# chanzuckerberg/saber

Hardware: AMD Instinct MI355X
Metric: EM slices/sec (1024^2, Hiera-L) (higher is better)
Workload: dtype bf16; 1 GPU; 1024x1024 uint16 EM slice -> prep.prepare -> SAM2 AMG (Hiera-L, cfgAMG defaults: npoints=32, crop_n_layers=2 -> 21 crops, 3072 grid prompts + 9216 m2m refinements, multimask) -> dedup/sort -> uint16 label plane; BASELINE configs[1]; weights=seeded synthetic Hiera-L (no checkpoint offline), slices_per_rank=22, engine_handles_per_gpu=2, parallelism=single GPU

## Files before the change

include/saber_amd_kernels.h:

```cpp
#ifndef SABER_AMD_KERNELS_H
#define SABER_AMD_KERNELS_H
#include <stddef.h>
#include <stdint.h>
#ifdef __cplusplus
extern "C" {
#endif

const char* saber_k_last_error(void);
int saber_k_init(int device_id);

int saber_k_gemm(const uint16_t* A, const uint16_t* W, const float* bias, const float* res, float* out_f32, uint16_t* out_bf16,
                 int M, int N, int K, int act, int act_last, int pool4, int res_shift, int res_mod, void* stream);

int saber_k_gemm_ld(const uint16_t* A, int lda, const uint16_t* W, int ldw, int w_kpad, const float* bias, const float* res, float* out_f32,
                    uint16_t* out_bf16, int M, int N, int K, int act, void* stream);

int saber_k_gemm_rowln(const uint16_t* A, int lda, const uint16_t* W, int ldw, const float* bias, const float* res, float* out_f32,
                       uint16_t* out_bf16, const float* ln_gamma, const float* ln_beta, float ln_eps, uint16_t* ln_out, int M, int N, int K,
                       void* stream);

int saber_k_mlp_rowln(const uint16_t* A, int lda, const uint16_t* W1, int ldw1, const float* b1, const uint16_t* W2, int ldw2, const float* b2,
                      const float* res, float* out_f32, uint16_t* out_bf16, const float* ln_gamma, const float* ln_beta, float ln_eps,
                      uint16_t* ln_out, int M, int C, void* stream);

// ... 1 lines not shown
                      int rows, int C, int act, void* stream);

int saber_k_hiera_attention(const uint16_t* qkv, uint16_t* out, int n_windows, int nk, int heads, int q_pool, void* stream);
int saber_k_hiera_attention_ex(const uint16_t* qkv, uint16_t* out, int n_windows, int nk, int heads, int head_dim, int q_pool,
                               const uint8_t* key_mask, void* stream);

int saber_k_dec_attention(const float* q, const float* k, const float* v, uint16_t* out, int B, int nq, int nk, int heads, int hd,
                          int k_shared, void* stream);

int saber_k_prepare(const void* img, int dtype, int H, int W, float* out, float* ws_dev, uint32_t* minmax_dev, void* stream);

int saber_k_mask_post(const float* lowres, int n, int crop_x0, int crop_y0, int crop_w, int crop_h, int H, int W, float thr,
                      float offset, uint32_t* bits, int32_t* stats, void* stream);
int saber_k_mask_post_ex(const float* lowres, const int* idx, const uint8_t* pass, int n, int crop_x0, int crop_y0, int crop_w, int crop_h,
                         int H, int W, float thr, float offset, uint32_t* bits, int32_t* stats, void* stream);

int saber_k_resize_normalize(const float* img, int H, int W, int channels, const int* crops_dev, int n, float* out, int res, void* stream);
int saber_k_patch_embed(const float* pix, const float* wt, const float* bias, const float* pos, float* out, int n_images, int C, void* stream);

int saber_k_rope(const float* x, int64_t rows, int n_rot, int C, int side, float theta, float* out_f32, uint16_t* out_bf16, void* stream);
int saber_k_softmax_rows(const float* S, int64_t ld_s, int64_t rows, int n, float scale, uint16_t* P, int64_t ld_p, void* stream);
int saber_k_conv3x3s2(const float* in, int H, int W, int Cin, const float* w, const float* b, int Cout, float* out, void* stream);
int saber_k_conv3x3s2_t(const float* in, int H, int W, int Cin, const float* wt, const float* b, int Cout, float* out, void* stream);
int saber_k_paint_nearest(const float* logits, int Hv, int Wv, float thr, int label, uint16_t* plane, int H, int W, int* any_flag, void* stream);
int saber_k_paint_nearest_stack(const float* logits, int n, int Hv, int Wv, const int* labels_host, float thr, uint16_t* plane, int H, int W,
                                int* any_flag, void* stream);
int saber_k_relabel_frames(uint16_t* vol, int Z, int64_t HW, const uint16_t* lut, int L, void* stream);
int saber_k_merge_max_u16(uint16_t* acc, const uint16_t* src, int64_t n, int binarize, void* stream);
int saber_k_merge_class_conf(uint16_t* final_labels, float* best, const uint16_t* src, const uint16_t* cls, const float* conf, int L, int64_t n,
                             void* stream);
// ... 105 lines not shown
```

saber_amd/_lib.py:

```python
import ctypes as C
import os
import subprocess

_HERE = os.path.dirname(os.path.abspath(__file__))
LIB_PATH = os.path.join(_HERE, "libsaber_amd.so")
CSRC = os.path.join(_HERE, "csrc")


class SaberAmdError(RuntimeError):
    pass


class SaberRangeError(SaberAmdError):
    """SABER_ERR_RANGE: the engine's overflow sentinel found NaN / inf in the 16-bit arithmetic (include/saber_amd.h:
    saber_engine_check_finite) - with fp16 operands, an activation beyond 65 504.  The call's results are invalid."""


SABER_OK, SABER_ERR_INVALID, SABER_ERR_STATE, SABER_ERR_HIP, SABER_ERR_CAPACITY, SABER_ERR_RANGE = 0, -1, -2, -3, -4, -5


def build(verbose: bool = False) -> str:
    r = subprocess.run(["make", "-C", CSRC, "-j8"], capture_output=True, text=True)
    if r.returncode != 0:
        raise SaberAmdError("building libsaber_amd.so failed:\n" + r.stdout[-4000:] + r.stderr[-4000:])
# ... 105 lines not shown
    "saber_encoder_flops": (C.c_double, [_vp]),
    "saber_decoder_flops_per_prompt": (C.c_double, []),
    "saber_k_last_error": (C.c_char_p, []),
    "saber_k_init": (_i, [_i]),
    "saber_k_gemm": (_i, [_vp, _vp, _vp, _vp, _vp, _vp, _i, _i, _i, _i, _i, _i, _i, _i, _vp]),
    "saber_k_gemm_ld": (_i, [_vp, _i, _vp, _i, _i, _vp, _vp, _vp, _vp, _i, _i, _i, _i, _vp]),
    "saber_k_gemm_rowln": (_i, [_vp, _i, _vp, _i, _vp, _vp, _vp, _vp, _vp, _vp, _f, _vp, _i, _i, _i, _vp]),
    "saber_k_mlp_rowln": (_i, [_vp, _i, _vp, _i, _vp, _vp, _i, _vp, _vp, _vp, _vp, _vp, _vp, _f, _vp, _i, _i, _vp]),
    "saber_k_layernorm": (_i, [_vp, _vp, _vp, _f, _vp, _vp, _i, _i, _i, _vp]),
    "saber_k_hiera_attention": (_i, [_vp, _vp, _i, _i, _i, _i, _vp]),
    "saber_k_hiera_attention_ex": (_i, [_vp, _vp, _i, _i, _i, _i, _i, _vp, _vp]),
    "saber_k_dec_attention": (_i, [_vp, _vp, _vp, _vp, _i, _i, _i, _i, _i, _i, _vp]),
    "saber_k_prepare": (_i, [_vp, _i, _i, _i, _vp, _vp, _vp, _vp]),
    "saber_k_mask_post": (_i, [_vp, _i, _i, _i, _i, _i, _i, _i, _f, _f, _vp, _vp, _vp]),
    "saber_k_mask_post_ex": (_i, [_vp, _vp, _vp, _i, _i, _i, _i, _i, _i, _i, _f, _f, _vp, _vp, _vp]),
    "saber_k_resize_normalize": (_i, [_vp, _i, _i, _i, _vp, _i, _vp, _i, _vp]),
    "saber_k_patch_embed": (_i, [_vp, _vp, _vp, _vp, _vp, _i, _i, _vp]),
    "saber_k_perm_index": (_i, [_i, _i, _i]),
    "saber_k_set_operand_type": (_i, [_i]),
    "saber_k_stream_create_cu_range": (_i, [_i, _i, C.POINTER(_vp)]),
    "saber_k_stream_destroy": (_i, [_vp]),
    "saber_k_host_f32_to_f16": (None, [_vp, _vp, C.c_int64]),
    "saber_k_dec_i2t": (_i, [_vp, C.c_int64, _vp, _vp, _vp, _f, _vp, _vp, _vp, _vp, _vp, _f, _vp, _i, _vp]),
    "saber_k_dec_i2t16": (_i, [_vp, C.c_int64, _vp, _vp, _vp, _f, _vp, _vp, _vp, _vp, _vp, _f, _vp, _i, _i, _vp]),
    "saber_k_dec_t2i": (_i, [_vp, C.c_int64, _vp, _vp, _vp, _f, _vp, _vp, _i, _i, _vp, _vp, _vp, _vp]),
    "saber_k_dec_upscale": (_i, [_vp, _vp, _vp, _vp, _vp, _vp, _vp, _vp, _vp, _i, _i, _vp, _vp, _i, _vp, _vp, _i, _vp, _vp]),
    "saber_k_hyper_pack": (_i, [_vp, _i, _vp, _vp, _vp]),
    "saber_k_mask_pick": (_i, [_vp, _vp, _i, _i, _vp, _vp, _vp, _vp]),
    "saber_k_mask_select": (_i, [_vp, _vp, _i, _i, _vp, _vp, _vp]),
    "saber_k_iou_live_flags": (_i, [_vp, _i, _f, _vp, _vp, _vp]),
# ... 79 lines not shown
```

saber_amd/csrc/amg.hip:

```cpp
#include <algorithm>
#include <array>
#include <cmath>
#include <numeric>

#include "common.h"
#include "engine.h"

#define TRY(x) do { int _r = (x); if (_r != SABER_OK) return _r; } while (0)

struct Cand {
    float box[4];
    float iou, stab;
    float pt[2];
    int crop[4];
    int area;
    size_t bits_slot;
};

static std::vector<int> nms_host(const std::vector<Cand>& c, const std::vector<float>& scores, float thr) {
    const int n = (int)c.size();
    std::vector<int> order(n);
    std::iota(order.begin(), order.end(), 0);
    std::stable_sort(order.begin(), order.end(), [&](int a, int b) { return scores[a] > scores[b]; });
    std::vector<char> sup(n, 0);
// ... 238 lines not shown
            if (prm->use_m2m) {
                float* pts2 = e->amg_pts2 + 2 * gr.k0;
                float* low2 = e->amg_low2 + gr.k0 * 4 * 65536;
                float* iou2 = e->amg_iou2 + gr.k0;
                int* sel2 = e->amg_sel + gr.k0;
                TRY(eng_graphed(e, "dec2," + key_of({ci, nm, (long long)(uintptr_t)pts2, G * nm, first_raw, (long long)(uintptr_t)low1, (long long)(uintptr_t)low2, (long long)(uintptr_t)iou2, (long long)(uintptr_t)sel2,
                                                     (long long)(e->iou_prune ? std::lround(prm->pred_iou_thresh * 1e6f) + 1 : 0)}), s,
                                [&]() { return eng_decode_ex(e, ci, nm, pts2, nullptr, G * nm, 0, low1, first_raw, 32.0f, low2, 1, iou2, nullptr, sel2, s, prm->pred_iou_thresh); }));
                for (int g = 0; g < G; ++g) e->slot_embb_valid[ci + g] = 1;
                gr.masks = low2; gr.ious = iou2; gr.plane_mode = 2;
            }
        }
        if (use_dev) {
            const float* iou_all = prm->use_m2m ? e->amg_iou2 : e->amg_iou1;
            std::vector<DevCrop> dcs;
            for (const Grp& gr : groups) {
                ENG_KP(e, PC_ELEMENTWISE, 0.0, 0.0, launch_amg_plane(iou_all + gr.k0, gr.plane_mode == 2 ? e->amg_sel + gr.k0 : nullptr, gr.G * gr.nm, gr.plane_mode, prm->pred_iou_thresh,
                                                                  e->amg_idx + gr.k0, e->amg_pass + gr.k0, s));
                if (lowres_clean)
                    ENG_KP(e, PC_MASK_POST, 0.0, 0.0, launch_clean_lowres(const_cast<float*>(gr.masks), e->amg_idx + gr.k0, e->amg_pass + gr.k0, gr.G * gr.nm, 256, 256, prm->mask_threshold,
                                                                         e->lowres_hole_area, e->lowres_sprinkle_area, s));
                for (int g = 0; g < gr.G; ++g) {
                    const auto& box = crops[c0 + gr.ci + g];
                    DevCrop dc{{box[0], box[1], box[2], box[3]}, (int)(gr.k0 + (size_t)g * gr.nm), gr.nm, (int)(gr.pt0 + (size_t)g * gr.np), M};
                    dcs.push_back(dc);
                    ENG_KP(e, PC_MASK_POST, 0.0, (double)gr.nm * (65536.0 * 4 + (double)mask_words * 4),
                           launch_mask_post(gr.masks, e->amg_idx + dc.kbase, gr.nm, box[0], box[1], box[2] - box[0], box[3] - box[1], H, W, prm->mask_threshold,
                                            prm->stability_score_offset, e->amg_crop_bits + (slot_base + dc.kbase) * mask_words, e->amg_stats + dc.kbase, s, e->amg_pass + dc.kbase));
                }
            }
            ENG_HIP(e, hipMemcpyAsync(e->amg_crops_dev, dcs.data(), sizeof(DevCrop) * dcs.size(), hipMemcpyHostToDevice, s));
            ENG_HIP(e, hipMemcpyAsync(e->amg_crop_pts, crop_pts_all.data(), sizeof(float) * 2 * n_pts, hipMemcpyHostToDevice, s));
            ENG_KP(e, PC_MASK_POST, 0.0, 0.0, launch_amg_crops(e->amg_crops_dev, (int)dcs.size(), max_nm, e->amg_stats, e->amg_pass, iou_all, e->amg_crop_pts, prm->stability_score_thresh,
                                                            prm->box_nms_thresh, H, W, (int)slot_base, e->amg_tmp, e->amg_keep, e->amg_counts, e->amg_surv, e->amg_nsurv, (int)total_cand, s));
            slot_base += n_cand;
            continue;
        }
        std::vector<float> h_iou_all(n_cand);
        std::vector<int> h_sel;
        ENG_HIP(e, hipMemcpyAsync(h_iou_all.data(), prm->use_m2m ? e->amg_iou2 : e->amg_iou1, sizeof(float) * n_cand, hipMemcpyDeviceToHost, s));
        if (prm->use_m2m) { h_sel.resize(n_cand); ENG_HIP(e, hipMemcpyAsync(h_sel.data(), e->amg_sel, sizeof(int) * n_cand, hipMemcpyDeviceToHost, s)); }
        { ENG_HIP(e, hipStreamSynchronize(s)); ++e->amg_last_syncs; }
        struct CropRange { int first, count; };
        std::vector<std::vector<CropRange>> ranges(groups.size());
        h_idx.clear();
        for (size_t gi = 0; gi < groups.size(); ++gi) {
// ... 165 lines not shown
```

saber_amd/csrc/capi_kernels.hip:

```cpp
#include <cmath>
#include <cstring>
#include <string>
#include <vector>

#include "../../include/saber_amd_kernels.h"
#include "common.h"
#include "kernels.h"
#include "engine.h"
#include "exact.h"

#include <atomic>

static thread_local std::string g_kerr;
static int kfail(const char* m) { g_kerr = m ? m : "unknown"; return -1; }
static int kcheck(const char* m) {
    if (m) return kfail(m);
    hipError_t st = hipGetLastError();
    if (st != hipSuccess) return kfail(hipGetErrorString(st));
    return 0;
}

extern "C" const char* saber_k_last_error(void) { return g_kerr.c_str(); }

extern "C" int saber_k_init(int device_id) {
// ... 104 lines not shown
    if (dtype == 0) return kcheck(launch_prepare_u16((const uint16_t*)img, H, W, out, ws_dev, minmax_dev, (hipStream_t)stream));
    if (dtype == 1) return kcheck(launch_prepare_f32((const float*)img, H, W, out, ws_dev, minmax_dev, (hipStream_t)stream));
    return kfail("prepare: dtype must be 0 (u16) or 1 (f32)");
}

extern "C" int saber_k_mask_post(const float* lowres, int n, int crop_x0, int crop_y0, int crop_w, int crop_h, int H, int W, float thr,
                                 float offset, uint32_t* bits, int32_t* stats, void* stream) {
    return kcheck(launch_mask_post(lowres, nullptr, n, crop_x0, crop_y0, crop_w, crop_h, H, W, thr, offset, bits,
                                   reinterpret_cast<MaskStats*>(stats), (hipStream_t)stream));
}

extern "C" int saber_k_mask_post_ex(const float* lowres, const int* idx, const uint8_t* pass, int n, int crop_x0, int crop_y0, int crop_w, int crop_h,
                                    int H, int W, float thr, float offset, uint32_t* bits, int32_t* stats, void* stream) {
    return kcheck(launch_mask_post(lowres, idx, n, crop_x0, crop_y0, crop_w, crop_h, H, W, thr, offset, bits,
                                   reinterpret_cast<MaskStats*>(stats), (hipStream_t)stream, pass));
}

extern "C" int saber_k_resize_normalize(const float* img, int H, int W, int channels, const int* crops_dev, int n, float* out, int res, void* stream) {
    if (res <= 0 || (res % 16) != 0) return kfail("resize_normalize: res must be a positive multiple of 16");
    if (n <= 0) return 0;
    return kcheck(launch_resize_normalize(img, H, W, channels, crops_dev, n, out, res, (hipStream_t)stream));
}

extern "C" int saber_k_patch_embed(const float* pix, const float* wt, const float* bias, const float* pos, float* out, int n_images, int C, void* stream) {
    if (n_images <= 0) return 0;
    return kcheck(launch_patch_embed(pix, wt, bias, pos, out, n_images, C, 1024, (hipStream_t)stream));
}

extern "C" int saber_k_perm_index(int y, int x, int stage) { return perm_index(y, x, stage); }

// ... 327 lines not shown
```

saber_amd/csrc/decoder_ops.hip:

```cpp
#include <algorithm>

#include "common.h"
#include "kernels.h"

#define DEC_C 256

__global__ __launch_bounds__(256) void prompt_tokens_kernel(const float* __restrict__ pts, const int* __restrict__ labels, int P,
                                                            PromptWeights w, float* __restrict__ tokens) {
    const int p = blockIdx.x, c = threadIdx.x;
    float* t = tokens + (int64_t)p * 8 * DEC_C;
#pragma unroll
    for (int k = 0; k < 6; ++k) t[k * DEC_C + c] = w.out_tokens[k * DEC_C + c];
    const int label = labels ? labels[p] : 1;
    float e = 0.f;
    if (label >= 0) {
        const float x = 2.0f * ((pts[2 * p] + 0.5f) / 1024.0f) - 1.0f;
        const float y = 2.0f * ((pts[2 * p + 1] + 0.5f) / 1024.0f) - 1.0f;
        const int f = c & 127;
        const float a = 6.283185307179586f * (x * w.gauss[f] + y * w.gauss[128 + f]);
        e = (c < 128 ? sinf(a) : cosf(a)) + w.point_embed[(label & 3) * DEC_C + c];
    } else {
        e = w.not_a_point[c];
    }
    t[6 * DEC_C + c] = e;
// ... 691 lines not shown
        for (int w = 0; w < 4; ++w) {
            a += red[w][0]; in_ += red[w][1]; u += red[w][2];
            x0 = min(x0, red[w][3]); x1 = max(x1, red[w][4]); y0 = min(y0, red[w][5]); y1 = max(y1, red[w][6]);
        }
        MaskStats* st = stats + mi;
        if (a) {
            atomicAdd(&st->area, a);
            atomicMin(&st->x0, x0); atomicMax(&st->x1, x1);
            atomicMin(&st->y0, y0); atomicMax(&st->y1, y1);
        }
        if (in_) atomicAdd(&st->inter, in_);
        if (u) atomicAdd(&st->uni, u);
    }
}

__global__ __launch_bounds__(256) void mask_post_w1k_kernel(const float* __restrict__ lowres, const int* __restrict__ idx, int crop_x0,
                                                            int crop_y0, int crop_w, int crop_h, int H, int W, float thr, float offset,
                                                            uint32_t* __restrict__ bits, MaskStats* __restrict__ stats, const uint8_t* __restrict__ pass) {
    if (pass && !pass[blockIdx.y]) return;
    __shared__ float vrow[4][260];
    __shared__ int red[4][8];
    const int mi = blockIdx.y;
    const float* src = lowres + (int64_t)(idx ? idx[mi] : mi) * 65536;
    const int lane = threadIdx.x & 63, wave = threadIdx.x >> 6;
    const int W32 = (W + 31) >> 5;
    const float sy_scale = 256.0f / (float)crop_h, sx_scale = 256.0f / (float)crop_w;
    const int c_lo = max(crop_x0, 0) >> 6, c_hi = min(crop_x0 + crop_w - 1, W - 1) >> 6;
    int x0a[16];
    float lxa[16];
#pragma unroll
    for (int c = 0; c < 16; ++c) {
        const int x = 64 * c + lane, cx = x - crop_x0;
        float sx = ((float)cx + 0.5f) * sx_scale - 0.5f;
        sx = fmaxf(sx, 0.f);
        const int x0i = min((int)sx, 255);
        const bool valid = x < W && cx >= 0 && cx < crop_w;
        x0a[c] = valid ? x0i : 257;
        lxa[c] = valid ? sx - (float)x0i : 0.0f;
    }
    if (lane < 2) vrow[wave][257 + lane] = -3.0e38f;
    auto fetch = [&](int y, float4* a, float4* b, float* ly) -> bool {
        const int cy = y - crop_y0;
        if (y >= H || cy < 0 || cy >= crop_h) return false;
        float sy = ((float)cy + 0.5f) * sy_scale - 0.5f;
        sy = fmaxf(sy, 0.f);
        const int y0i = min((int)sy, 255), y1i = min(y0i + 1, 255);
        *ly = sy - (float)y0i;
        *a = *reinterpret_cast<const float4*>(src + y0i * 256 + lane * 4);
        *b = *reinterpret_cast<const float4*>(src + y1i * 256 + lane * 4);
        return true;
    };
    int area = 0, inter = 0, uni = 0, xmin = 1 << 30, xmax = -1, ymin = 1 << 30, ymax = -1;
    const int ybase = blockIdx.x * MP_ROWS + wave * (MP_ROWS / 4);
    float4 na = make_float4(0.f, 0.f, 0.f, 0.f), nb = na;
    float nly = 0.f;
    bool nin = fetch(ybase, &na, &nb, &nly);
    for (int r = 0; r < MP_ROWS / 4; ++r) {
        const int y = ybase + r;
        if (y >= H) break;
        uint32_t* brow = bits + ((int64_t)mi * H + y) * W32;
        const float4 a = na, b = nb;
        const float ly = nly;
        const bool in_crop = nin;
        nin = (r + 1 < MP_ROWS / 4) ? fetch(y + 1, &na, &nb, &nly) : false;
        if (!in_crop) {
            for (int wd = lane; wd < W32; wd += 64) brow[wd] = 0u;
            continue;
        }
        __builtin_amdgcn_wave_barrier();
        {
            float* vw = vrow[wave] + lane * 4;
            vw[0] = (1.0f - ly) * a.x + ly * b.x; vw[1] = (1.0f - ly) * a.y + ly * b.y;
            vw[2] = (1.0f - ly) * a.z + ly * b.z; vw[3] = (1.0f - ly) * a.w + ly * b.w;
            if (lane == 63) vw[4] = vw[3];
        }
        __builtin_amdgcn_wave_barrier();
        const float* vr = vrow[wave];
        uint32_t blo = 0u, bhi = 0u;
        float ta[16], tb[16];
#pragma unroll
        for (int cc = 0; cc < 16; ++cc) { ta[cc] = vr[x0a[cc]]; tb[cc] = vr[x0a[cc] + 1]; }
#define MP_CHUNK(cc)                                                                                              \
        if ((cc) >= c_lo && (cc) <= c_hi) {                                                                       \
            const float lx = lxa[cc];                                                                             \
            const float v = (1.0f - lx) * ta[cc] + lx * tb[cc];                                                   \
            const unsigned long long bm = __ballot(v > thr);                                                      \
            asm("s_nop 1\n\tv_writelane_b32 %0, %1, " #cc : "+v"(blo) : "s"((uint32_t)bm));     \
            asm("v_writelane_b32 %0, %1, " #cc : "+v"(bhi) : "s"((uint32_t)(bm >> 32)));                          \
            inter += (v > thr + offset) ? 1 : 0;                                                                  \
            uni += (v > thr - offset) ? 1 : 0;                                                                    \
        }
        MP_CHUNK(0) MP_CHUNK(1) MP_CHUNK(2) MP_CHUNK(3) MP_CHUNK(4) MP_CHUNK(5) MP_CHUNK(6) MP_CHUNK(7)
        MP_CHUNK(8) MP_CHUNK(9) MP_CHUNK(10) MP_CHUNK(11) MP_CHUNK(12) MP_CHUNK(13) MP_CHUNK(14) MP_CHUNK(15)
#undef MP_CHUNK
        const int pc = __popc(blo) + __popc(bhi);
        area += pc;
        if (pc) {
            xmin = min(xmin, lane * 64 + (blo ? __ffs((int)blo) - 1 : 31 + __ffs((int)bhi)));
            xmax = max(xmax, lane * 64 + (bhi ? 63 - __clz((int)bhi) : 31 - __clz((int)blo)));
        }
        if (__ballot(pc != 0)) { ymin = min(ymin, y); ymax = max(ymax, y); }
        const int wd = lane * 2;
        if (wd < W32) brow[wd] = blo;
        if (wd + 1 < W32) brow[wd + 1] = bhi;
    }
#pragma unroll
    for (int o = 32; o > 0; o >>= 1) {
        area += __shfl_xor(area, o, 64); inter += __shfl_xor(inter, o, 64); uni += __shfl_xor(uni, o, 64);
        xmin = min(xmin, __shfl_xor(xmin, o, 64)); xmax = max(xmax, __shfl_xor(xmax, o, 64));
    }
    if (lane == 0) {
        red[wave][0] = area; red[wave][1] = inter; red[wave][2] = uni; red[wave][3] = xmin;
        red[wave][4] = xmax; red[wave][5] = ymin; red[wave][6] = ymax;
    }
    __syncthreads();
    if (threadIdx.x == 0) {
        int a = 0, in_ = 0, u = 0, x0 = 1 << 30, x1 = -1, y0 = 1 << 30, y1 = -1;
        for (int w = 0; w < 4; ++w) {
            a += red[w][0]; in_ += red[w][1]; u += red[w][2];
            x0 = min(x0, red[w][3]); x1 = max(x1, red[w][4]); y0 = min(y0, red[w][5]); y1 = max(y1, red[w][6]);
        }
        MaskStats* st = stats + mi;
        if (a) {
            atomicAdd(&st->area, a);
            atomicMin(&st->x0, x0); atomicMax(&st->x1, x1);
            atomicMin(&st->y0, y0); atomicMax(&st->y1, y1);
        }
        if (in_) atomicAdd(&st->inter, in_);
        if (u) atomicAdd(&st->uni, u);
    }
}

__global__ void mask_stats_init_kernel(MaskStats* stats, int n) {
    const int i = blockIdx.x * 256 + threadIdx.x;
    if (i < n) { MaskStats s; s.area = 0; s.inter = 0; s.uni = 0; s.x0 = 1 << 30; s.y0 = 1 << 30; s.x1 = -1; s.y1 = -1; s.pad = 0; stats[i] = s; }
}

const char* launch_mask_post(const float* lowres, const int* idx, int n, int crop_x0, int crop_y0, int crop_w, int crop_h, int H,
                             int W, float thr, float offset, uint32_t* bits, MaskStats* stats, hipStream_t s, const uint8_t* pass) {
    if (n <= 0) return nullptr;
    if (crop_w <= 0 || crop_h <= 0) return "mask_post: empty crop";
    hipLaunchKernelGGL(mask_stats_init_kernel, dim3((n + 255) / 256), dim3(256), 0, s, stats, n);
    const dim3 grid((H + MP_ROWS - 1) / MP_ROWS, n);
    if (W <= 1024 && !(g_saber_debug_flags & 8)) hipLaunchKernelGGL(mask_post_w1k_kernel, grid, dim3(256), 0, s, lowres, idx, crop_x0, crop_y0, crop_w, crop_h, H, W, thr, offset, bits, stats, pass);
    else if (W <= 1024) hipLaunchKernelGGL(mask_post_kernel<true>, grid, dim3(256), 0, s, lowres, idx, crop_x0, crop_y0, crop_w, crop_h, H, W, thr, offset, bits, stats, pass);
    else hipLaunchKernelGGL(mask_post_kernel<false>, grid, dim3(256), 0, s, lowres, idx, crop_x0, crop_y0, crop_w, crop_h, H, W, thr, offset, bits, stats, pass);
    return nullptr;
}

__global__ __launch_bounds__(256) void label_plane_kernel(const uint32_t* __restrict__ bits, const int* __restrict__ order, int n, int H,
                                                          int W, uint16_t* __restrict__ plane) {
    const int W32 = (W + 31) >> 5;
    const int64_t words = (int64_t)H * W32;
    for (int64_t wi = (int64_t)blockIdx.x * 256 + threadIdx.x; wi < words; wi += (int64_t)gridDim.x * 256) {
        const int y = (int)(wi / W32), xw = (int)(wi - (int64_t)y * W32);
        uint16_t lab[32];
#pragma unroll
        for (int b = 0; b < 32; ++b) lab[b] = 0;
        for (int i = 0; i < n; ++i) {
            const int mi = order ? order[i] : i;
            const uint32_t wd = bits[(int64_t)mi * words + wi];
// ... 172 lines not shown
```

saber_amd/csrc/kernels.h:

```cpp
#pragma once
#include <hip/hip_runtime.h>
#include <stdint.h>
#include <stddef.h>

extern int g_saber_debug_flags;
extern unsigned long long* g_saber_stamp_buf;
int saber_cu_count();
extern thread_local int g_saber_op_f16;
inline bool saber_op_is_f16() { return g_saber_op_f16 != 0; }

typedef uint16_t bf16_t;

enum { ACT_NONE = 0, ACT_GELU = 1, ACT_RELU = 2, ACT_SIGMOID = 3 };

struct GemmParams {
    const bf16_t* A = nullptr; int64_t lda = 0; int64_t strideA = 0;
    const bf16_t* W = nullptr; int64_t ldw = 0; int64_t strideW = 0;
    const float* bias = nullptr; int64_t strideBias = 0;
    const float* res = nullptr; int64_t ldres = 0; int64_t strideRes = 0;
    float* Cf = nullptr; int64_t ldcf = 0; int64_t strideCf = 0;
    bf16_t* Cb = nullptr; int64_t ldcb = 0; int64_t strideCb = 0;
    int M = 0, N = 0, K = 0;
    int act = ACT_NONE;
    int act_last = 0;
// ... 143 lines not shown
#define SABER_OP_FWD(fn)                                                                                                  \
    template <class... A> inline auto fn(A&&... a) {                                                                      \
        return saber_op_is_f16() ? op_f16::fn(static_cast<A&&>(a)...) : op_bf16::fn(static_cast<A&&>(a)...);              \
    }
#define SABER_OP_INIT(fn)                                                                                                 \
    inline const char* fn() { const char* m = op_bf16::fn(); return m ? m : op_f16::fn(); }
SABER_OP_INIT(gemm_init_device) SABER_OP_INIT(gemm_rowln_init_device) SABER_OP_INIT(gemm_mlp_rowln_init_device) SABER_OP_INIT(hiera_attention_init_device)
SABER_OP_INIT(decoder_fused_init_device) SABER_OP_INIT(decoder_tokens_init_device) SABER_OP_INIT(decoder_t16_init_device)
SABER_OP_FWD(launch_gemm) SABER_OP_FWD(gemm_rowln_supported) SABER_OP_FWD(launch_gemm_rowln) SABER_OP_FWD(gemm_rowln_packed_elems) SABER_OP_FWD(launch_pack_w_kstep)
SABER_OP_FWD(gemm_mlp_rowln_width) SABER_OP_FWD(gemm_mlp_rowln_packed_elems) SABER_OP_FWD(launch_pack_mlp_chunks) SABER_OP_FWD(launch_gemm_mlp_rowln)
SABER_OP_FWD(launch_layernorm) SABER_OP_FWD(launch_gather_rows) SABER_OP_FWD(launch_add_to_bf16) SABER_OP_FWD(launch_hiera_attention)
SABER_OP_FWD(launch_prompt_tokens) SABER_OP_FWD(launch_prompt_tokens_multi) SABER_OP_FWD(launch_mask_embed_src) SABER_OP_FWD(launch_mask_hidden) SABER_OP_FWD(launch_embb_tiles)
SABER_OP_FWD(launch_dec_attention) SABER_OP_FWD(launch_mask_pick) SABER_OP_FWD(launch_iou_live_flags) SABER_OP_FWD(launch_mask_select)
SABER_OP_FWD(launch_dec_t2i) SABER_OP_FWD(launch_dec_i2t) SABER_OP_FWD(launch_dec_upscale) SABER_OP_FWD(launch_hyper_pack) SABER_OP_FWD(launch_dec_tokens)
SABER_OP_FWD(launch_prompt_tokens16) SABER_OP_FWD(launch_dec_tokens16) SABER_OP_FWD(launch_dec_i2t16)
SABER_OP_FWD(launch_mask_post) SABER_OP_FWD(launch_gather_masks) SABER_OP_FWD(launch_label_plane) SABER_OP_FWD(launch_pair_intersections) SABER_OP_FWD(launch_unpermute_nchw)
SABER_OP_FWD(launch_rope) SABER_OP_FWD(launch_softmax_rows) SABER_OP_FWD(launch_conv3x3s2) SABER_OP_FWD(launch_unpack_masks) SABER_OP_FWD(launch_paint_nearest)
SABER_OP_FWD(launch_conv3x3s2_t) SABER_OP_FWD(launch_dwconv7_t) SABER_OP_FWD(launch_dwconv7) SABER_OP_FWD(launch_conv4x4s4) SABER_OP_FWD(launch_resize_plane)
SABER_OP_FWD(launch_resize_planes_non_overlap)
SABER_OP_FWD(launch_flash256) SABER_OP_FWD(launch_gauss_mirror) SABER_OP_FWD(launch_axpy) SABER_OP_FWD(launch_bf16_to_f32)
SABER_OP_FWD(launch_rope_batched) SABER_OP_FWD(launch_flash256_batched) SABER_OP_FWD(launch_membank_assemble)
SABER_OP_FWD(launch_conv3x3s2_t_batched) SABER_OP_FWD(launch_dwconv7_t_batched)
#undef SABER_OP_FWD
#undef SABER_OP_INIT
#endif
```

saber_amd/csrc/kernels_op.h:

```cpp
const char* launch_gemm(const GemmParams& p, hipStream_t stream);
const char* gemm_init_device();
bool gemm_rowln_supported(const GemmParams& p);
const char* launch_gemm_rowln(const GemmParams& p, hipStream_t stream);
const char* gemm_rowln_init_device();
size_t gemm_rowln_packed_elems(int N, int K);
const char* launch_pack_w_kstep(const bf16_t* W, int ldw, int N, int K, bf16_t* out, hipStream_t s);
bool gemm_mlp_rowln_width(int C);
size_t gemm_mlp_rowln_packed_elems(int C);
const char* launch_pack_mlp_chunks(const bf16_t* W1, int ldw1, const bf16_t* W2, int ldw2, int C, bf16_t* out, hipStream_t s);
const char* launch_gemm_mlp_rowln(const GemmParams& p, hipStream_t stream);
const char* gemm_mlp_rowln_init_device();
const char* launch_layernorm(const LayerNormParams& p, hipStream_t s);
const char* launch_gather_rows(const float* in, int64_t in_rows, float* out, int64_t out_rows, const int* idx, int C, int n_images, hipStream_t s);
const char* launch_add_to_bf16(const float* x, const float* y, int ymod, bf16_t* out_bf, float* out_f, int64_t rows, int C,
                               hipStream_t s);
const char* launch_hiera_attention(const bf16_t* qkv, bf16_t* out, int n_windows, int nk, int heads, int hd, int q_pool,
                                   const uint8_t* kmask, hipStream_t s);
const char* hiera_attention_init_device();
const char* launch_prompt_tokens(const float* pts, const int* labels, int P, PromptWeights w, float* tokens, hipStream_t s);
const char* launch_prompt_tokens_multi(const float* pts, const int* labels, int P, int K, PromptWeights w, float* tokens, hipStream_t s);
const char* launch_mask_embed_src(const float* mask_in, int P, const float* image_embed, XMap emb_map, const float* pos, MaskEmbedWeights w,
                                  float* src_f, bf16_t* src_bf, bf16_t* srcpos_bf, float clamp_abs, hipStream_t s, int raw4_q0 = -1);
const char* launch_mask_hidden(const float* mask_in, int P, MaskEmbedWeights w, bf16_t* h2, float clamp_abs, hipStream_t s, int raw4_q0 = -1);
const char* launch_embb_tiles(const float* emb, const float* b3, float* out, hipStream_t s);
// ... 9 lines not shown
                           const float* bo, const float* gamma, const float* beta, float eps, bf16_t* Xout, int P, hipStream_t s, const XBuild* build = nullptr);
const char* launch_dec_upscale(const bf16_t* X, const bf16_t* W1, const float* b1, const float* ln_g, const float* ln_b, const bf16_t* W2p,
                               const float* b2, const float* fs1, const float* fs0, XMap slot_map, const float* hyper, const bf16_t* hyper_pk, float* masks4, int P,
                               hipStream_t s, const uint8_t* live = nullptr, const float* iou4 = nullptr, int multimask = 0, unsigned int* sentinel = nullptr);
const char* launch_hyper_pack(const float* hyper, int P, bf16_t* hyper_pk, unsigned int* counter, hipStream_t s);
const char* decoder_fused_init_device();
const char* launch_dec_tokens(const TokSeg& s, hipStream_t st);
const char* decoder_tokens_init_device();
const char* launch_prompt_tokens16(const float* pts, const int* labels, int P, int K, PromptWeights w, float* tokens, hipStream_t s);
const char* launch_dec_tokens16(const TokSeg& s, int nvalid, hipStream_t st);
const char* launch_dec_i2t16(const bf16_t* X, XMap xm, const bf16_t* peq, const bf16_t* Kt, const float* tk, float kscale, const float* cb, const bf16_t* VtT,
                             const float* bo, const float* gamma, const float* beta, float eps, bf16_t* Xout, int P, int nvalid, hipStream_t s);
const char* decoder_t16_init_device();
const char* launch_mask_post(const float* lowres, const int* idx, int n, int crop_x0, int crop_y0, int crop_w, int crop_h, int H,
                             int W, float thr, float offset, uint32_t* bits, MaskStats* stats, hipStream_t s, const uint8_t* pass = nullptr);
const char* launch_gather_masks(const uint32_t* src, const int* idx, uint32_t* dst, int n, int64_t words, hipStream_t s);
const char* launch_label_plane(const uint32_t* bits, const int* order, int n, int H, int W, uint16_t* plane, hipStream_t s);
const char* launch_pair_intersections(const uint32_t* bits, int n, int64_t words, int* inter, hipStream_t s);
const char* launch_unpermute_nchw(const float* tok, int C, int stage, float* out, hipStream_t s);
const char* launch_rope(const float* x, int64_t rows, int n_rot, int C, int side, float theta, float* out_f, bf16_t* out_bf, hipStream_t s);
const char* launch_rope_batched(const float* x, int64_t rows_per, int batch, int n_rot, int C, int side, float theta, float* out_f, bf16_t* out_bf, hipStream_t s);
const char* launch_softmax_rows(const float* S, int64_t lds_, int64_t rows, int n, float scale, bf16_t* P, int64_t ldp, hipStream_t s);
const char* launch_conv3x3s2(const float* in, int H, int W, int Cin, const float* w, const float* b, int Cout, float* out, hipStream_t s);
const char* launch_unpack_masks(const uint32_t* bits, int n, int H, int W, uint8_t* out, hipStream_t s);
const char* launch_paint_nearest(const float* logits, int Hv, int Wv, float thr, int label, uint16_t* plane, int H, int W, int* any_flag, hipStream_t s);
const char* launch_conv3x3s2_t(const float* in, int H, int W, int Cin, const float* wt, const float* b, int Cout, float* out, hipStream_t s);
const char* launch_dwconv7_t(const float* in, int H, int W, int C, const float* wt, const float* b, float* out, hipStream_t s);
const char* launch_conv3x3s2_t_batched(const float* in, int64_t in_stride, int H, int W, int Cin, const float* wt, const float* b, int Cout, float* out,
                                       int64_t out_stride, int batch, hipStream_t s);
const char* launch_dwconv7_t_batched(const float* in, int64_t in_stride, int H, int W, int C, const float* wt, const float* b, float* out, int64_t out_stride,
// ... 16 lines not shown
```

Baseline: 7.649 slices/s.

## Batch mask post-processing across crops in one launch with band-skipping and LDS-staged bit writes

Replaces the per-crop mask_post launches with a single grouped launch per group, using a device crop table that each block searches to find its crop box. The crop table upload moves ahead of the launches. Row bands and per-wave row ranges that fall outside the crop now just zero their output, and the horizontal tap table is built once per block in shared memory. A WIDE variant stages the bit rows in LDS and writes them out as 16-byte vector stores. This cuts launch count and wasted work on out-of-crop rows, at the cost of extra shared memory and a linear crop search per block.

```diff
diff --git a/include/saber_amd_kernels.h b/include/saber_amd_kernels.h
--- a/include/saber_amd_kernels.h
+++ b/include/saber_amd_kernels.h
@@ -39,6 +39,9 @@
                       float offset, uint32_t* bits, int32_t* stats, void* stream);
 int saber_k_mask_post_ex(const float* lowres, const int* idx, const uint8_t* pass, int n, int crop_x0, int crop_y0, int crop_w, int crop_h,
                          int H, int W, float thr, float offset, uint32_t* bits, int32_t* stats, void* stream);
+
+int saber_k_mask_post_group(const float* lowres, const int* idx, const uint8_t* pass, const int32_t* crops_host, const int32_t* crops_dev, int n_crops,
+                            int H, int W, float thr, float offset, uint32_t* bits, int32_t* stats, void* stream);
 
 int saber_k_resize_normalize(const float* img, int H, int W, int channels, const int* crops_dev, int n, float* out, int res, void* stream);
 int saber_k_patch_embed(const float* pix, const float* wt, const float* bias, const float* pos, float* out, int n_images, int C, void* stream);
diff --git a/saber_amd/_lib.py b/saber_amd/_lib.py
--- a/saber_amd/_lib.py
+++ b/saber_amd/_lib.py
@@ -143,6 +143,7 @@
     "saber_k_prepare": (_i, [_vp, _i, _i, _i, _vp, _vp, _vp, _vp]),
     "saber_k_mask_post": (_i, [_vp, _i, _i, _i, _i, _i, _i, _i, _f, _f, _vp, _vp, _vp]),
     "saber_k_mask_post_ex": (_i, [_vp, _vp, _vp, _i, _i, _i, _i, _i, _i, _i, _f, _f, _vp, _vp, _vp]),
+    "saber_k_mask_post_group": (_i, [_vp, _vp, _vp, _vp, _vp, _i, _i, _i, _f, _f, _vp, _vp, _vp]),
     "saber_k_resize_normalize": (_i, [_vp, _i, _i, _i, _vp, _i, _vp, _i, _vp]),
     "saber_k_patch_embed": (_i, [_vp, _vp, _vp, _vp, _vp, _i, _i, _vp]),
     "saber_k_perm_index": (_i, [_i, _i, _i]),
diff --git a/saber_amd/csrc/amg.hip b/saber_amd/csrc/amg.hip
--- a/saber_amd/csrc/amg.hip
+++ b/saber_amd/csrc/amg.hip
@@ -276,22 +276,24 @@
         if (use_dev) {
             const float* iou_all = prm->use_m2m ? e->amg_iou2 : e->amg_iou1;
             std::vector<DevCrop> dcs;
+            for (const Grp& gr : groups)
+                for (int g = 0; g < gr.G; ++g) {
+                    const auto& box = crops[c0 + gr.ci + g];
+                    dcs.push_back(DevCrop{{box[0], box[1], box[2], box[3]}, (int)(gr.k0 + (size_t)g * gr.nm), gr.nm, (int)(gr.pt0 + (size_t)g * gr.np), M});
+                }
+            ENG_HIP(e, hipMemcpyAsync(e->amg_crops_dev, dcs.data(), sizeof(DevCrop) * dcs.size(), hipMemcpyHostToDevice, s));
+            size_t dc0 = 0;
             for (const Grp& gr : groups) {
                 ENG_KP(e, PC_ELEMENTWISE, 0.0, 0.0, launch_amg_plane(iou_all + gr.k0, gr.plane_mode == 2 ? e->amg_sel + gr.k0 : nullptr, gr.G * gr.nm, gr.plane_mode, prm->pred_iou_thresh,
                                                                   e->amg_idx + gr.k0, e->amg_pass + gr.k0, s));
                 if (lowres_clean)
                     ENG_KP(e, PC_MASK_POST, 0.0, 0.0, launch_clean_lowres(const_cast<float*>(gr.masks), e->amg_idx + gr.k0, e->amg_pass + gr.k0, gr.G * gr.nm, 256, 256, prm->mask_threshold,
                                                                          e->lowres_hole_area, e->lowres_sprinkle_area, s));
-                for (int g = 0; g < gr.G; ++g) {
-                    const auto& box = crops[c0 + gr.ci + g];
-                    DevCrop dc{{box[0], box[1], box[2], box[3]}, (int)(gr.k0 + (size_t)g * gr.nm), gr.nm, (int)(gr.pt0 + (size_t)g * gr.np), M};
-                    dcs.push_back(dc);
-                    ENG_KP(e, PC_MASK_POST, 0.0, (double)gr.nm * (65536.0 * 4 + (double)mask_words * 4),
-                           launch_mask_post(gr.masks, e->amg_idx + dc.kbase, gr.nm, box[0], box[1], box[2] - box[0], box[3] - box[1], H, W, prm->mask_threshold,
-                                            prm->stability_score_offset, e->amg_crop_bits + (slot_base + dc.kbase) * mask_words, e->amg_stats + dc.kbase, s, e->amg_pass + dc.kbase));
-                }
-            }
-            ENG_HIP(e, hipMemcpyAsync(e->amg_crops_dev, dcs.data(), sizeof(DevCrop) * dcs.size(), hipMemcpyHostToDevice, s));
+                ENG_KP(e, PC_MASK_POST, 0.0, (double)gr.G * gr.nm * (65536.0 * 4 + (double)mask_words * 4),
+                       launch_mask_post_group(gr.masks, e->amg_idx + gr.k0, e->amg_crops_dev + dc0, dcs.data() + dc0, gr.G, H, W, prm->mask_threshold, prm->stability_score_offset,
+                                              e->amg_crop_bits + (slot_base + gr.k0) * mask_words, e->amg_stats + gr.k0, s, e->amg_pass + gr.k0));
+                dc0 += (size_t)gr.G;
+            }
             ENG_HIP(e, hipMemcpyAsync(e->amg_crop_pts, crop_pts_all.data(), sizeof(float) * 2 * n_pts, hipMemcpyHostToDevice, s));
             ENG_KP(e, PC_MASK_POST, 0.0, 0.0, launch_amg_crops(e->amg_crops_dev, (int)dcs.size(), max_nm, e->amg_stats, e->amg_pass, iou_all, e->amg_crop_pts, prm->stability_score_thresh,
                                                             prm->box_nms_thresh, H, W, (int)slot_base, e->amg_tmp, e->amg_keep, e->amg_counts, e->amg_surv, e->amg_nsurv, (int)total_cand, s));
diff --git a/saber_amd/csrc/capi_kernels.hip b/saber_amd/csrc/capi_kernels.hip
--- a/saber_amd/csrc/capi_kernels.hip
+++ b/saber_amd/csrc/capi_kernels.hip
@@ -142,6 +142,14 @@
                                     int H, int W, float thr, float offset, uint32_t* bits, int32_t* stats, void* stream) {
     return kcheck(launch_mask_post(lowres, idx, n, crop_x0, crop_y0, crop_w, crop_h, H, W, thr, offset, bits,
                                    reinterpret_cast<MaskStats*>(stats), (hipStream_t)stream, pass));
+}
+
+extern "C" int saber_k_mask_post_group(const float* lowres, const int* idx, const uint8_t* pass, const int32_t* crops_host, const int32_t* crops_dev, int n_crops,
+                                       int H, int W, float thr, float offset, uint32_t* bits, int32_t* stats, void* stream) {
+    static_assert(sizeof(DevCrop) == 8 * sizeof(int32_t), "saber_k_mask_post_group: 8 int32 per crop");
+    if (n_crops > 0 && (!crops_host || !crops_dev)) return kfail("mask_post_group: the crop table is needed on the host and on the device");
+    return kcheck(launch_mask_post_group(lowres, idx, reinterpret_cast<const DevCrop*>(crops_dev), reinterpret_cast<const DevCrop*>(crops_host), n_crops, H, W, thr, offset,
+                                         bits, reinterpret_cast<MaskStats*>(stats), (hipStream_t)stream, pass));
 }
 
 extern "C" int saber_k_resize_normalize(const float* img, int H, int W, int channels, const int* crops_dev, int n, float* out, int res, void* stream) {
diff --git a/saber_amd/csrc/decoder_ops.hip b/saber_amd/csrc/decoder_ops.hip
--- a/saber_amd/csrc/decoder_ops.hip
+++ b/saber_amd/csrc/decoder_ops.hip
@@ -729,100 +729,148 @@
     }
 }
 
-__global__ __launch_bounds__(256) void mask_post_w1k_kernel(const float* __restrict__ lowres, const int* __restrict__ idx, int crop_x0,
-                                                            int crop_y0, int crop_w, int crop_h, int H, int W, float thr, float offset,
+template <bool WIDE>
+__global__ __launch_bounds__(256, 4) void mask_post_w1k_kernel(const float* __restrict__ lowres, const int* __restrict__ idx, const DevCrop* __restrict__ crops,
+                                                            int n_crops, int crop_x0, int crop_y0, int crop_w, int crop_h, int H, int W, float thr, float offset,
                                                             uint32_t* __restrict__ bits, MaskStats* __restrict__ stats, const uint8_t* __restrict__ pass) {
     if (pass && !pass[blockIdx.y]) return;
+    const int mi = blockIdx.y;
+    if (crops) {
+        const int k = crops[0].kbase + mi;
+        int c = 0;
+        while (c < n_crops && (k < crops[c].kbase || k >= crops[c].kbase + crops[c].nm)) ++c;
+        if (c == n_crops) return;
+        crop_x0 = crops[c].box[0]; crop_y0 = crops[c].box[1]; crop_w = crops[c].box[2] - crop_x0; crop_h = crops[c].box[3] - crop_y0;
+    }
     __shared__ float vrow[4][260];
     __shared__ int red[4][8];
-    const int mi = blockIdx.y;
+    __shared__ int2 tap[1024];
+    __shared__ __attribute__((aligned(16))) uint32_t wbits[WIDE ? 4 : 1][WIDE ? 512 : 4];
     const float* src = lowres + (int64_t)(idx ? idx[mi] : mi) * 65536;
     const int lane = threadIdx.x & 63, wave = threadIdx.x >> 6;
     const int W32 = (W + 31) >> 5;
+    const int band = (int)((blockIdx.x + blockIdx.y) % gridDim.x);
+    const int ybase = band * MP_ROWS + wave * (MP_ROWS / 4);
+    auto zero_rows = [&](int y, int nr) {
+        if (WIDE) {
+            uint4* dst = reinterpret_cast<uint4*>(bits + ((int64_t)mi * H + y) * W32);
+            for (int q = lane; q < nr * (W32 >> 2); q += 64) dst[q] = make_uint4(0u, 0u, 0u, 0u);
+        } else {
+            for (int r = 0; r < nr; ++r) {
+                uint32_t* brow = bits + ((int64_t)mi * H + y + r) * W32;
+                for (int wd = lane; wd < W32; wd += 64) brow[wd] = 0u;
+            }
+        }
+    };
+    const int wave_rows = min(MP_ROWS / 4, H - ybase);
+    if (band * MP_ROWS >= crop_y0 + crop_h || band * MP_ROWS + MP_ROWS <= crop_y0) {
+        if (wave_rows > 0) zero_rows(ybase, wave_rows);
+        return;
+    }
     const float sy_scale = 256.0f / (float)crop_h, sx_scale = 256.0f / (float)crop_w;
     const int c_lo = max(crop_x0, 0) >> 6, c_hi = min(crop_x0 + crop_w - 1, W - 1) >> 6;
-    int x0a[16];
-    float lxa[16];
-#pragma unroll
-    for (int c = 0; c < 16; ++c) {
-        const int x = 64 * c + lane, cx = x - crop_x0;
+    for (int x = 64 * c_lo + (int)threadIdx.x; x < 64 * c_hi + 64; x += 256) {
+        const int cx = x - crop_x0;
         float sx = ((float)cx + 0.5f) * sx_scale - 0.5f;
         sx = fmaxf(sx, 0.f);
         const int x0i = min((int)sx, 255);
         const bool valid = x < W && cx >= 0 && cx < crop_w;
-        x0a[c] = valid ? x0i : 257;
-        lxa[c] = valid ? sx - (float)x0i : 0.0f;
+        tap[x] = make_int2(valid ? x0i : 257, __float_as_int(valid ? sx - (float)x0i : 0.0f));
     }
     if (lane < 2) vrow[wave][257 + lane] = -3.0e38f;
-    auto fetch = [&](int y, float4* a, float4* b, float* ly) -> bool {
-        const int cy = y - crop_y0;
-        if (y >= H || cy < 0 || cy >= crop_h) return false;
-        float sy = ((float)cy + 0.5f) * sy_scale - 0.5f;
-        sy = fmaxf(sy, 0.f);
-        const int y0i = min((int)sy, 255), y1i = min(y0i + 1, 255);
-        *ly = sy - (float)y0i;
-        *a = *reinterpret_cast<const float4*>(src + y0i * 256 + lane * 4);
-        *b = *reinterpret_cast<const float4*>(src + y1i * 256 + lane * 4);
-        return true;
-    };
+    __syncthreads();
     int area = 0, inter = 0, uni = 0, xmin = 1 << 30, xmax = -1, ymin = 1 << 30, ymax = -1;
-    const int ybase = blockIdx.x * MP_ROWS + wave * (MP_ROWS / 4);
-    float4 na = make_float4(0.f, 0.f, 0.f, 0.f), nb = na;
-    float nly = 0.f;
-    bool nin = fetch(ybase, &na, &nb, &nly);
-    for (int r = 0; r < MP_ROWS / 4; ++r) {
-        const int y = ybase + r;
-        if (y >= H) break;
-        uint32_t* brow = bits + ((int64_t)mi * H + y) * W32;
-        const float4 a = na, b = nb;
-        const float ly = nly;
-        const bool in_crop = nin;
-        nin = (r + 1 < MP_ROWS / 4) ? fetch(y + 1, &na, &nb, &nly) : false;
-        if (!in_crop) {
-            for (int wd = lane; wd < W32; wd += 64) brow[wd] = 0u;
-            continue;
-        }
-        __builtin_amdgcn_wave_barrier();
-        {
-            float* vw = vrow[wave] + lane * 4;
-            vw[0] = (1.0f - ly) * a.x + ly * b.x; vw[1] = (1.0f - ly) * a.y + ly * b.y;
-            vw[2] = (1.0f - ly) * a.z + ly * b.z; vw[3] = (1.0f - ly) * a.w + ly * b.w;
-            if (lane == 63) vw[4] = vw[3];
-        }
-        __builtin_amdgcn_wave_barrier();
-        const float* vr = vrow[wave];
-        uint32_t blo = 0u, bhi = 0u;
-        float ta[16], tb[16];
-#pragma unroll
-        for (int cc = 0; cc < 16; ++cc) { ta[cc] = vr[x0a[cc]]; tb[cc] = vr[x0a[cc] + 1]; }
+    if (wave_rows > 0 && (ybase >= crop_y0 + crop_h || ybase + MP_ROWS / 4 <= crop_y0)) {
+        zero_rows(ybase, wave_rows);
+    } else if (wave_rows > 0) {
+        int x0a[16];
+        float lxa[16];
+#pragma unroll
+        for (int c = 0; c < 16; ++c) {
+            x0a[c] = 257; lxa[c] = 0.0f;
+            if (c >= c_lo && c <= c_hi) { const int2 t = tap[64 * c + lane]; x0a[c] = t.x; lxa[c] = __int_as_float(t.y); }
+        }
+        auto fetch = [&](int y, float4* a, float4* b, float* ly) -> bool {
+            const int cy = y - crop_y0;
+            if (y >= H || cy < 0 || cy >= crop_h) return false;
+            float sy = ((float)cy + 0.5f) * sy_scale - 0.5f;
+            sy = fmaxf(sy, 0.f);
+            const int y0i = min((int)sy, 255), y1i = min(y0i + 1, 255);
+            *ly = sy - (float)y0i;
+            *a = *reinterpret_cast<const float4*>(src + y0i * 256 + lane * 4);
+            *b = *reinterpret_cast<const float4*>(src + y1i * 256 + lane * 4);
+            return true;
+        };
+        float4 na = make_float4(0.f, 0.f, 0.f, 0.f), nb = na;
+        float nly = 0.f;
+        bool nin = fetch(ybase, &na, &nb, &nly);
+#pragma unroll 1
+        for (int r = 0; r < MP_ROWS / 4; ++r) {
+            const int y = ybase + r;
+            if (y >= H) break;
+            uint32_t* brow = bits + ((int64_t)mi * H + y) * W32;
+            uint32_t* wrow = wbits[WIDE ? wave : 0] + (WIDE ? r * W32 : 0);
+            const float4 a = na, b = nb;
+            const float ly = nly;
+            const bool in_crop = nin;
+            nin = (r + 1 < MP_ROWS / 4) ? fetch(y + 1, &na, &nb, &nly) : false;
+            if (!in_crop) {
+                if (WIDE) { if (2 * lane < W32) *reinterpret_cast<uint2*>(wrow + 2 * lane) = make_uint2(0u, 0u); }
+                else for (int wd = lane; wd < W32; wd += 64) brow[wd] = 0u;
+                continue;
+            }
+            __builtin_amdgcn_wave_barrier();
+            {
+                float* vw = vrow[wave] + lane * 4;
+                vw[0] = (1.0f - ly) * a.x + ly * b.x; vw[1] = (1.0f - ly) * a.y + ly * b.y;
+                vw[2] = (1.0f - ly) * a.z + ly * b.z; vw[3] = (1.0f - ly) * a.w + ly * b.w;
+                if (lane == 63) vw[4] = vw[3];
+            }
+            __builtin_amdgcn_wave_barrier();
+            const float* vr = vrow[wave];
+            uint32_t blo = 0u, bhi = 0u;
+            float ta[16], tb[16];
+#pragma unroll
+            for (int cc = 0; cc < 16; ++cc) { ta[cc] = vr[x0a[cc]]; tb[cc] = vr[x0a[cc] + 1]; }
 #define MP_CHUNK(cc)                                                                                              \
-        if ((cc) >= c_lo && (cc) <= c_hi) {                                                                       \
-            const float lx = lxa[cc];                                                                             \
-            const float v = (1.0f - lx) * ta[cc] + lx * tb[cc];                                                   \
-            const unsigned long long bm = __ballot(v > thr);                                                      \
-            asm("s_nop 1\n\tv_writelane_b32 %0, %1, " #cc : "+v"(blo) : "s"((uint32_t)bm));     \
-            asm("v_writelane_b32 %0, %1, " #cc : "+v"(bhi) : "s"((uint32_t)(bm >> 32)));                          \
-            inter += (v > thr + offset) ? 1 : 0;                                                                  \
-            uni += (v > thr - offset) ? 1 : 0;                                                                    \
-        }
-        MP_CHUNK(0) MP_CHUNK(1) MP_CHUNK(2) MP_CHUNK(3) MP_CHUNK(4) MP_CHUNK(5) MP_CHUNK(6) MP_CHUNK(7)
-        MP_CHUNK(8) MP_CHUNK(9) MP_CHUNK(10) MP_CHUNK(11) MP_CHUNK(12) MP_CHUNK(13) MP_CHUNK(14) MP_CHUNK(15)
+            if ((cc) >= c_lo && (cc) <= c_hi) {                                                                   \
+                const float lx = lxa[cc];                                                                         \
+                const float v = (1.0f - lx) * ta[cc] + lx * tb[cc];                                               \
+                const unsigned long long bm = __ballot(v > thr);                                                  \
+                asm("s_nop 1\n\tv_writelane_b32 %0, %1, " #cc : "+v"(blo) : "s"((uint32_t)bm));     \
+                asm("v_writelane_b32 %0, %1, " #cc : "+v"(bhi) : "s"((uint32_t)(bm >> 32)));                      \
+                inter += (v > thr + offset) ? 1 : 0;                                                              \
+                uni += (v > thr - offset) ? 1 : 0;                                                                \
+            }
+            MP_CHUNK(0) MP_CHUNK(1) MP_CHUNK(2) MP_CHUNK(3) MP_CHUNK(4) MP_CHUNK(5) MP_CHUNK(6) MP_CHUNK(7)
+            MP_CHUNK(8) MP_CHUNK(9) MP_CHUNK(10) MP_CHUNK(11) MP_CHUNK(12) MP_CHUNK(13) MP_CHUNK(14) MP_CHUNK(15)
 #undef MP_CHUNK
-        const int pc = __popc(blo) + __popc(bhi);
-        area += pc;
-        if (pc) {
-            xmin = min(xmin, lane * 64 + (blo ? __ffs((int)blo) - 1 : 31 + __ffs((int)bhi)));
-            xmax = max(xmax, lane * 64 + (bhi ? 63 - __clz((int)bhi) : 31 - __clz((int)blo)));
-        }
-        if (__ballot(pc != 0)) { ymin = min(ymin, y); ymax = max(ymax, y); }
-        const int wd = lane * 2;
-        if (wd < W32) brow[wd] = blo;
-        if (wd + 1 < W32) brow[wd + 1] = bhi;
-    }
-#pragma unroll
-    for (int o = 32; o > 0; o >>= 1) {
-        area += __shfl_xor(area, o, 64); inter += __shfl_xor(inter, o, 64); uni += __shfl_xor(uni, o, 64);
-        xmin = min(xmin, __shfl_xor(xmin, o, 64)); xmax = max(xmax, __shfl_xor(xmax, o, 64));
+            const int pc = __popc(blo) + __popc(bhi);
+            area += pc;
+            if (pc) {
+                xmin = min(xmin, lane * 64 + (blo ? __ffs((int)blo) - 1 : 31 + __ffs((int)bhi)));
+                xmax = max(xmax, lane * 64 + (bhi ? 63 - __clz((int)bhi) : 31 - __clz((int)blo)));
+            }
+            if (__ballot(pc != 0)) { ymin = min(ymin, y); ymax = max(ymax, y); }
+            if (WIDE) {
+                if (2 * lane < W32) *reinterpret_cast<uint2*>(wrow + 2 * lane) = make_uint2(blo, bhi);
+            } else {
+                const int wd = lane * 2;
+                if (wd < W32) brow[wd] = blo;
+                if (wd + 1 < W32) brow[wd + 1] = bhi;
+            }
+        }
+        if (WIDE) {
+            __builtin_amdgcn_wave_barrier();
+            uint4* dst = reinterpret_cast<uint4*>(bits + ((int64_t)mi * H + ybase) * W32);
+            const uint4* wsrc = reinterpret_cast<const uint4*>(wbits[WIDE ? wave : 0]);
+            for (int q = lane; q < wave_rows * (W32 >> 2); q += 64) dst[q] = wsrc[q];
+        }
+#pragma unroll
+        for (int o = 32; o > 0; o >>= 1) {
+            area += __shfl_xor(area, o, 64); inter += __shfl_xor(inter, o, 64); uni += __shfl_xor(uni, o, 64);
+            xmin = min(xmin, __shfl_xor(xmin, o, 64)); xmax = max(xmax, __shfl_xor(xmax, o, 64));
+        }
     }
     if (lane == 0) {
         red[wave][0] = area; red[wave][1] = inter; red[wave][2] = uni; red[wave][3] = xmin;
@@ -851,15 +899,48 @@
     if (i < n) { MaskStats s; s.area = 0; s.inter = 0; s.uni = 0; s.x0 = 1 << 30; s.y0 = 1 << 30; s.x1 = -1; s.y1 = -1; s.pad = 0; stats[i] = s; }
 }
 
+static void mask_post_w1k(const float* lowres, const int* idx, const DevCrop* crops, int n_crops, int n, int crop_x0, int crop_y0, int crop_w, int crop_h, int H, int W,
+                          float thr, float offset, uint32_t* bits, MaskStats* stats, hipStream_t s, const uint8_t* pass) {
+    const dim3 grid((H + MP_ROWS - 1) / MP_ROWS, n);
+    const bool wide = (((W + 31) >> 5) & 3) == 0 && (reinterpret_cast<uintptr_t>(bits) & 15) == 0;
+    if (wide) hipLaunchKernelGGL(mask_post_w1k_kernel<true>, grid, dim3(256), 0, s, lowres, idx, crops, n_crops, crop_x0, crop_y0, crop_w, crop_h, H, W, thr, offset, bits, stats, pass);
+    else hipLaunchKernelGGL(mask_post_w1k_kernel<false>, grid, dim3(256), 0, s, lowres, idx, crops, n_crops, crop_x0, crop_y0, crop_w, crop_h, H, W, thr, offset, bits, stats, pass);
+}
+
 const char* launch_mask_post(const float* lowres, const int* idx, int n, int crop_x0, int crop_y0, int crop_w, int crop_h, int H,
                              int W, float thr, float offset, uint32_t* bits, MaskStats* stats, hipStream_t s, const uint8_t* pass) {
     if (n <= 0) return nullptr;
     if (crop_w <= 0 || crop_h <= 0) return "mask_post: empty crop";
     hipLaunchKernelGGL(mask_stats_init_kernel, dim3((n + 255) / 256), dim3(256), 0, s, stats, n);
     const dim3 grid((H + MP_ROWS - 1) / MP_ROWS, n);
-    if (W <= 1024 && !(g_saber_debug_flags & 8)) hipLaunchKernelGGL(mask_post_w1k_kernel, grid, dim3(256), 0, s, lowres, idx, crop_x0, crop_y0, crop_w, crop_h, H, W, thr, offset, bits, stats, pass);
+    if (W <= 1024 && !(g_saber_debug_flags & 8)) mask_post_w1k(lowres, idx, nullptr, 0, n, crop_x0, crop_y0, crop_w, crop_h, H, W, thr, offset, bits, stats, s, pass);
     else if (W <= 1024) hipLaunchKernelGGL(mask_post_kernel<true>, grid, dim3(256), 0, s, lowres, idx, crop_x0, crop_y0, crop_w, crop_h, H, W, thr, offset, bits, stats, pass);
     else hipLaunchKernelGGL(mask_post_kernel<false>, grid, dim3(256), 0, s, lowres, idx, crop_x0, crop_y0, crop_w, crop_h, H, W, thr, offset, bits, stats, pass);
+    return nullptr;
+}
+
+const char* launch_mask_post_group(const float* lowres, const int* idx, const DevCrop* crops_dev, const DevCrop* crops_host, int n_crops, int H, int W, float thr,
+                                   float offset, uint32_t* bits, MaskStats* stats, hipStream_t s, const uint8_t* pass) {
+    if (n_crops <= 0) return nullptr;
+    int n = 0;
+    for (int c = 0; c < n_crops; ++c) {
+        const DevCrop& dc = crops_host[c];
+        if (dc.nm <= 0 || dc.kbase != crops_host[0].kbase + n) return "mask_post_group: the crops' candidates are not consecutive";
+        if (dc.box[2] <= dc.box[0] || dc.box[3] <= dc.box[1]) return "mask_post: empty crop";
+        n += dc.nm;
+    }
+    if (W > 1024 || (g_saber_debug_flags & (8 | 131072))) {
+        const int64_t words = (int64_t)H * ((W + 31) >> 5);
+        for (int c = 0; c < n_crops; ++c) {
+            const DevCrop& dc = crops_host[c];
+            const int off = dc.kbase - crops_host[0].kbase;
+            if (const char* m = launch_mask_post(idx ? lowres : lowres + (int64_t)off * 65536, idx ? idx + off : nullptr, dc.nm, dc.box[0], dc.box[1], dc.box[2] - dc.box[0],
+                                                 dc.box[3] - dc.box[1], H, W, thr, offset, bits + off * words, stats + off, s, pass ? pass + off : nullptr)) return m;
+        }
+        return nullptr;
+    }
+    hipLaunchKernelGGL(mask_stats_init_kernel, dim3((n + 255) / 256), dim3(256), 0, s, stats, n);
+    mask_post_w1k(lowres, idx, crops_dev, n_crops, n, 0, 0, 0, 0, H, W, thr, offset, bits, stats, s, pass);
     return nullptr;
 }
 
diff --git a/saber_amd/csrc/kernels.h b/saber_amd/csrc/kernels.h
--- a/saber_amd/csrc/kernels.h
+++ b/saber_amd/csrc/kernels.h
@@ -181,7 +181,7 @@
 SABER_OP_FWD(launch_dec_attention) SABER_OP_FWD(launch_mask_pick) SABER_OP_FWD(launch_iou_live_flags) SABER_OP_FWD(launch_mask_select)
 SABER_OP_FWD(launch_dec_t2i) SABER_OP_FWD(launch_dec_i2t) SABER_OP_FWD(launch_dec_upscale) SABER_OP_FWD(launch_hyper_pack) SABER_OP_FWD(launch_dec_tokens)
 SABER_OP_FWD(launch_prompt_tokens16) SABER_OP_FWD(launch_dec_tokens16) SABER_OP_FWD(launch_dec_i2t16)
-SABER_OP_FWD(launch_mask_post) SABER_OP_FWD(launch_gather_masks) SABER_OP_FWD(launch_label_plane) SABER_OP_FWD(launch_pair_intersections) SABER_OP_FWD(launch_unpermute_nchw)
+SABER_OP_FWD(launch_mask_post) SABER_OP_FWD(launch_mask_post_group) SABER_OP_FWD(launch_gather_masks) SABER_OP_FWD(launch_label_plane) SABER_OP_FWD(launch_pair_intersections) SABER_OP_FWD(launch_unpermute_nchw)
 SABER_OP_FWD(launch_rope) SABER_OP_FWD(launch_softmax_rows) SABER_OP_FWD(launch_conv3x3s2) SABER_OP_FWD(launch_unpack_masks) SABER_OP_FWD(launch_paint_nearest)
 SABER_OP_FWD(launch_conv3x3s2_t) SABER_OP_FWD(launch_dwconv7_t) SABER_OP_FWD(launch_dwconv7) SABER_OP_FWD(launch_conv4x4s4) SABER_OP_FWD(launch_resize_plane)
 SABER_OP_FWD(launch_resize_planes_non_overlap)
diff --git a/saber_amd/csrc/kernels_op.h b/saber_amd/csrc/kernels_op.h
--- a/saber_amd/csrc/kernels_op.h
+++ b/saber_amd/csrc/kernels_op.h
@@ -47,6 +47,8 @@
 const char* decoder_t16_init_device();
 const char* launch_mask_post(const float* lowres, const int* idx, int n, int crop_x0, int crop_y0, int crop_w, int crop_h, int H,
                              int W, float thr, float offset, uint32_t* bits, MaskStats* stats, hipStream_t s, const uint8_t* pass = nullptr);
+const char* launch_mask_post_group(const float* lowres, const int* idx, const DevCrop* crops_dev, const DevCrop* crops_host, int n_crops, int H, int W, float thr,
+                                   float offset, uint32_t* bits, MaskStats* stats, hipStream_t s, const uint8_t* pass = nullptr);
 const char* launch_gather_masks(const uint32_t* src, const int* idx, uint32_t* dst, int n, int64_t words, hipStream_t s);
 const char* launch_label_plane(const uint32_t* bits, const int* order, int n, int H, int W, uint16_t* plane, hipStream_t s);
 const char* launch_pair_intersections(const uint32_t* bits, int n, int64_t words, int* inter, hipStream_t s);
```

Result: faster. 7.731 slices/s (median of 6 runs) (+1.1%).
